# shengjie-chen/simple_image_compression_network

Measured on AMD Instinct MI355X. Metric: Mpixels/s encode+decode (4K RGB), higher is better.
Workload: dtype u8; 1 GPU; 8 x 3840x2160 RGB uint8 images per GPU, eight_layers_net (PARAM weights), BASELINE.json configs[3] shard; transform only (the reference has no coder); images_per_gpu=8, global_images=8, parallelism=image-sharded x1, partition=image i -> rank i mod world (dist.shard_indices)

## Files before the change

include/sicn.h:

```cpp
#ifndef SICN_H
#define SICN_H

#include <stddef.h>
#include <stdint.h>

#ifdef __cplusplus
extern "C" {
#endif

#define SICN_OK 0
#define SICN_EINVAL (-22)
#define SICN_ENOMEM (-12)
#define SICN_ENODEV (-19)
#define SICN_ENOSPC (-28)

typedef struct sicn_layer_desc {
    int32_t K;
    int32_t S;
    int32_t P;
    int32_t IFM_CH;
    int32_t IFM_ROW;
    int32_t IFM_COL;
    int32_t OFM_CH;
    int32_t OFM_ROW;
// ... 44 lines not shown
void sicn_weights_free(sicn_weights *w);

int sicn_conv2d(const sicn_layer_desc *desc, const sicn_weights *w, const uint8_t *in_nhwc,
                uint8_t *out_nhwc, int n_images, void *hip_stream);
int sicn_deconv522(const sicn_layer_desc *desc, const sicn_weights *w, const uint8_t *in_nhwc,
                   uint8_t *out_nhwc, int n_images, void *hip_stream);
int sicn_conv2d_opt(const sicn_layer_desc *desc, const sicn_weights *w, const uint8_t *in_nhwc,
                    uint8_t *out_nhwc, int n_images, const sicn_options *opt, void *hip_stream);
int sicn_deconv522_opt(const sicn_layer_desc *desc, const sicn_weights *w, const uint8_t *in_nhwc,
                       uint8_t *out_nhwc, int n_images, const sicn_options *opt, void *hip_stream);
const char *sicn_kernel_for(const sicn_layer_desc *desc);

int sicn_net_create(const sicn_layer_desc *descs, sicn_weights *const *weights, int n_layers,
                    sicn_net **out);
int sicn_net_create_opt(const sicn_layer_desc *descs, sicn_weights *const *weights, int n_layers,
                        const sicn_options *opt, sicn_net **out);
void sicn_net_free(sicn_net *net);
size_t sicn_net_workspace_bytes(const sicn_net *net, int n_images);
int sicn_net_forward(const sicn_net *net, int first_layer, int last_layer, const uint8_t *in,
                     uint8_t *out, int tap_layer, uint8_t *tap_out, int n_images, void *workspace,
                     size_t workspace_bytes, void *hip_stream);
int sicn_debug_net_columns(const sicn_net *net, int first_layer, int last_layer, int tap_layer, int n_images, int32_t *columns,
                           int32_t *live_outputs);
int sicn_eight_layers_net(const sicn_net *net, const uint8_t *in, uint8_t *out,
                          uint8_t *latent_or_null, int n_images, void *workspace,
                          size_t workspace_bytes, void *hip_stream);

int sicn_net_profile(sicn_net *net, int enable);
int sicn_net_layer_ms(sicn_net *net, int reset, float *ms_sum ,
                      int *launches );

#ifdef __cplusplus
}
#endif
#endif
```

simple_image_compression_network_amd/_lib.py:

```python
from __future__ import annotations

import ctypes
import os
from pathlib import Path

from .config import CLayerDesc

_PKG = Path(__file__).resolve().parent
LIB_PATH = Path(os.environ.get("SICN_LIB", _PKG / "libsicn.so"))

_vp, _i, _sz = ctypes.c_void_p, ctypes.c_int, ctypes.c_size_t


class COptions(ctypes.Structure):
    _fields_ = [(n, ctypes.c_int32) for n in ("struct_bytes", "force_generic", "mfma_shape", "tile_x", "strip_chunks",
                                              "no_phase_layout", "split_n", "wave_tile", "prefetch", "persistent_grid", "split_k", "l7_loader", "l0_form", "gdn_fuse")] + [("reserved", ctypes.c_int32 * 2)]


def make_options(**kw) -> "COptions":
    o = COptions()
    lib().sicn_options_init(ctypes.byref(o))
    for k, v in kw.items():
        if k not in dict(COptions._fields_) or k in ("struct_bytes", "reserved"):
            raise AttributeError(f"sicn_options has no field {k}")
# ... 8 lines not shown
    "sicn_strerror": (ctypes.c_char_p, [_i]),
    "sicn_validate_desc": (_i, [_descp]),
    "sicn_weights_from_finn_tiles": (_i, [_descp, _vp, _i, _vp, ctypes.POINTER(_vp)]),
    "sicn_weights_free": (None, [_vp]),
    "sicn_conv2d": (_i, [_descp, _vp, _vp, _vp, _i, _vp]),
    "sicn_deconv522": (_i, [_descp, _vp, _vp, _vp, _i, _vp]),
    "sicn_kernel_for": (ctypes.c_char_p, [_descp]),
    "sicn_options_init": (None, [ctypes.POINTER(COptions)]),
    "sicn_conv2d_opt": (_i, [_descp, _vp, _vp, _vp, _i, ctypes.POINTER(COptions), _vp]),
    "sicn_deconv522_opt": (_i, [_descp, _vp, _vp, _vp, _i, ctypes.POINTER(COptions), _vp]),
    "sicn_net_create_opt": (_i, [_descp, ctypes.POINTER(_vp), _i, ctypes.POINTER(COptions), ctypes.POINTER(_vp)]),
    "sicn_net_create": (_i, [_descp, ctypes.POINTER(_vp), _i, ctypes.POINTER(_vp)]),
    "sicn_net_free": (None, [_vp]),
    "sicn_net_workspace_bytes": (_sz, [_vp, _i]),
    "sicn_net_forward": (_i, [_vp, _i, _i, _vp, _vp, _i, _vp, _i, _vp, _sz, _vp]),
    "sicn_eight_layers_net": (_i, [_vp, _vp, _vp, _vp, _i, _vp, _sz, _vp]),
    "sicn_net_profile": (_i, [_vp, _i]),
    "sicn_net_layer_ms": (_i, [_vp, _i, ctypes.POINTER(ctypes.c_float), ctypes.POINTER(_i)]),
    "sicn_crop_nhwc": (_i, [_vp, _vp, _i, _i, _i, _i, _i, _i, _vp]),
    "sicn_debug_plan": (_i, [_descp, _i, ctypes.POINTER(COptions), _i, ctypes.POINTER(ctypes.c_int32)]),
    "sicn_debug_xcd_item": (ctypes.c_longlong, [ctypes.c_longlong, ctypes.c_longlong, _i]),
    "sicn_debug_chip": (_i, [ctypes.POINTER(ctypes.c_int32)]),
    "sicn_debug_net_columns": (_i, [_vp, _i, _i, _i, _i, ctypes.POINTER(ctypes.c_int32), ctypes.POINTER(ctypes.c_int32)]),
}


class CodecInfo(ctypes.Structure):
    _fields_ = [(n, ctypes.c_uint32) for n in ("mode", "image_width", "image_height", "lat_w", "lat_h", "lat_c",
                                               "n_symbols", "n_streams", "payload_bytes", "adler32", "stream_symbols")]


class CConvLayerDesc(ctypes.Structure):
    _fields_ = [(n, ctypes.c_int32) for n in ("K", "IFM_CH", "IFM_DIM", "OFM_CH", "OFM_DIM", "SIMD", "PE", "IN_BIT", "IN_SIGNED",
                                              "W_BIT", "W_TILES", "ACC_BIT", "ACC_SIGNED", "OUT_BIT", "activation", "NUM_TH",
                                              "ACT_VAL")]


_cldp = ctypes.POINTER(CConvLayerDesc)
CONVLAYER_ABI = {
    "sicn_convlayer_validate": (_i, [_cldp]),
    "sicn_convlayer_params_create": (_i, [_cldp, _vp, _i, _vp, ctypes.POINTER(_vp)]),
    "sicn_convlayer_params_free": (None, [_vp]),
    "sicn_conv_layer_batch": (_i, [_cldp, _vp, _vp, _vp, _i, _vp]),
    "sicn_conv_layer_batch_kernel": (_i, [_cldp, _vp, _vp, _vp, _i, _i, _vp]),
    "sicn_convlayer_kernel_for": (ctypes.c_char_p, [_cldp]),
}
# ... 201 lines not shown
```

simple_image_compression_network_amd/csrc/k_rgb.hip:

```cpp
#include <cstdlib>

#include <algorithm>

#include "k_l0_common.hpp"

namespace sicn {

template <int NTJ>
__global__ __launch_bounds__(256, 2) void k_l0(const uint8_t *__restrict__ in, uint8_t *__restrict__ out,
                                               const int8_t *__restrict__ w_l0,
                                               const int8_t *__restrict__ bias, int IW, int IH, int OW,
                                               int OH, int tiles_y, int ty_per, int out_layout, uint32_t act_floor)
{
    constexpr int COUT = NTJ * 32;
    constexpr int TB = COUT * KSTEP;
    constexpr int WBYTES = 5 * TB;
    extern __shared__ __attribute__((aligned(16))) uint8_t smem[];
    uint8_t *wl = smem;
    uint8_t *patch0 = smem + WBYTES;
    uint8_t *bias_lds = patch0 + 2 * L0_PATCH;
    uint8_t *raw = bias_lds + 128;

    const int tid = threadIdx.x, lane = tid & 63;
    const int w = __builtin_amdgcn_readfirstlane(tid >> 6);
// ... 127 lines not shown
        const size_t lds = 5 * 128 * KSTEP + 2 * L0_PATCH + 128 + L0_RAW_BYTES;
        hipError_t e = hipFuncSetAttribute((const void *)k_l0<4>, hipFuncAttributeMaxDynamicSharedMemorySize, (int)lds);
        if (e != hipSuccess) return e;
        hipLaunchKernelGGL(k_l0<4>, grid, dim3(256), lds, stream, in, out, w.d_w_l0, w.d_bias, g.IW, g.IH,
                           g.OW, g.OH, p.tiles_y, p.ty_per, out_layout,
                           (relu ? ACT_FLOOR_RELU : ACT_FLOOR_RAW) | (nt_store_wanted((size_t)g.OH * g.OW * g.COUT * n_images) ? ACT_NT_STORE : 0u));
    } else
        return hipErrorInvalidValue;
    return hipGetLastError();
}

constexpr int L7_AUX = 0;
constexpr int L7_PITCH = 36;
constexpr int L7_STEP_PIECES = L7_ROWS * L7_PITCH / 16;
constexpr int L7_AHEAD = 1;
constexpr int L7_RING_PIECES = ((4 * L7_AHEAD + 6) * L7_PITCH + 15) / 16;
constexpr int L7_WGS = 3;
constexpr int L7_RING_POS = L7_RING_PIECES * 16;
constexpr int L7_REGION = L7_RING_PIECES * 1024;
constexpr int L7_STAGE = 2 * 192;
constexpr int L7_X1 = 2 * 256;
constexpr int L7_X2 = 2 * 128;
constexpr int L7_XCH = 5 * L7_X1 + 4 * L7_X2;
constexpr int L7_LDS = 2 * L7_REGION + 4 * L7_STAGE + 1024 + L7_XCH;
constexpr int L7_KSTEPS = 6, L7_MTILES = 2;
static_assert(L7_ROWS * L7_PITCH % 16 == 0 && L7_RING_POS >= (4 * L7_AHEAD + 6) * L7_PITCH, "ring geometry");
static_assert(L7_WGS * L7_LDS <= 160 * 1024 && L7_XCH <= 4096, "three workgroups per CU");

template <int N>
__device__ __forceinline__ void l7_load_rows(uint8_t *patch, uint8_t *scratch, const uint8_t *in_img, int in_img_bytes, int w,
                                             int lane, int per_region, int iy0, int iy_min, int iy_max, int pslot0, int X0,
                                             int IW, const TensorMap &tm)
{
    __amdgpu_buffer_rsrc_t rs = __builtin_amdgcn_make_buffer_rsrc((void *)in_img, 0, in_img_bytes, 0x00020000);
    const int c2 = (lane & 3) ^ ((lane >> 4) & 3);
#pragma unroll
    for (int i = 0; i < N; i++) {
        const int j = w + 4 * i;
        const bool real = j < 2 * per_region;
        const int region = j >= per_region ? 1 : 0, kk = j - region * per_region;
        const int q = kk * 16 + (lane >> 2);
        const int row = q / L7_PITCH, tx = q - row * L7_PITCH;
        const int iy = iy0 + row, ix = X0 - 1 + tx;
        const bool ok = real && tx < TILE_X + 2 && iy >= iy_min && iy < iy_max && ix >= 0 && ix < IW;
        const uint32_t off = ok ? tensor_offset(tm, iy, ix, (uint32_t)(2 * region + (c2 >> 1))) + 16u * (c2 & 1) : OOB;
        int slot = pslot0 + kk;
        slot = slot >= L7_RING_PIECES ? slot - L7_RING_PIECES : slot;
        uint8_t *dst = real ? patch + region * L7_REGION + slot * 1024 : scratch;
        __builtin_amdgcn_raw_ptr_buffer_load_lds(rs, LDS_PTR(dst), 16, off, 0, 0, L7_AUX);
    }
}

__device__ __forceinline__ void l7_body(const uint8_t *__restrict__ in, uint8_t *__restrict__ out, const int8_t *__restrict__ w_l7,
                                        const int8_t *__restrict__ bias, int IW, int IH, int OW, int OH, int steps_y, int y_chunks,
                                        int tiles_x, int n_images, int in_layout, int n_xcd)
{
    constexpr int CIN = 128;
    extern __shared__ __attribute__((aligned(16))) uint8_t smem[];
    uint8_t *patch = smem;
    uint8_t *stage = smem + 2 * L7_REGION;
    uint8_t *scratch = stage + 4 * L7_STAGE;
    uint8_t *xch1 = scratch + 1024;
    uint8_t *xch2 = xch1 + 5 * L7_X1;

    const int tid = threadIdx.x, lane = tid & 63;
    const int w = __builtin_amdgcn_readfirstlane(tid >> 6);
    const int item = xcd_logical_index(tiles_x * y_chunks * n_images, n_xcd);
    if (item < 0) return;
    const int bx = item % tiles_x, by = (item / tiles_x) % y_chunks, img = item / (tiles_x * y_chunks);
    const int X0 = bx * TILE_X;
    const int per = (steps_y + y_chunks - 1) / y_chunks;
    const int s_begin = by * per, s_end = min(steps_y, s_begin + per);
    if (s_begin >= s_end) return;

    const int m = lane & 15, kg = lane >> 4;
    v4i wf[L7_MTILES * L7_KSTEPS];
#pragma unroll
    for (int s = 0; s < L7_MTILES * L7_KSTEPS; s++) wf[s] = *(const v4i *)(w_l7 + (s * 16 + m) * 64 + kg * 16);
    const int b0 = bias[0], b1 = bias[1], b2 = bias[2];

    const int in_img_bytes = IH * IW * CIN;
    const uint8_t *in_img = in + (size_t)img * in_img_bytes;
    uint8_t *out_img = out + (size_t)img * OH * OW * 3;
    const int py = kg >> 1, px = kg & 1;
    uint8_t *my_stage = stage + w * L7_STAGE;
    const bool fast_rows = ((OW * 3) & 3) == 0 && X0 + TILE_X <= IW;

    const int iy_top = 4 * s_begin - 3;
    const int iy_max = min(IH, 4 * s_end + 1);
    const TensorMap tm = tensor_map(in_layout, CIN, IW, IH);
    l7_load_rows<9>(patch, scratch, in_img, in_img_bytes, w, lane, 2 * L7_STEP_PIECES, iy_top, max(iy_top + 2, 0), iy_max, 0, X0,
                    IW, tm);
    int pnext = 2 * L7_STEP_PIECES;
    int ynext = iy_top + 8;
#pragma unroll
    for (int k = 1; k < L7_AHEAD; k++) {
        l7_load_rows<5>(patch, scratch, in_img, in_img_bytes, w, lane, L7_STEP_PIECES, ynext, 0, iy_max, pnext, X0, IW, tm);
        ynext += L7_ROWS;
        pnext += L7_STEP_PIECES;
        pnext = pnext >= L7_RING_PIECES ? pnext - L7_RING_PIECES : pnext;
    }

    auto frag_a = [&](int dx) { return (uint32_t)((4 + w) * L7_PITCH + m + dx); };
    auto frag_s = [&](uint32_t a) { return (uint32_t)((kg & 1) * L7_REGION) + ((((uint32_t)(kg >> 1)) ^ ((a >> 2) & 3u)) << 4); };
    uint32_t fa[3], fs[3];
#pragma unroll
    for (int dx = 0; dx < 3; dx++) {
        fa[dx] = frag_a(dx);
        fs[dx] = frag_s(fa[dx]);
    }
    const int w_below = (w + 1) & 3;
    const uint32_t x1_lane = (uint32_t)lane * 4u, x2_lane = (uint32_t)(px * 16 + m) * 4u;
    int saved[2][3] = {{0, 0, 0}, {0, 0, 0}};
    wait_vmcnt<5 * (L7_AHEAD - 1)>();
    block_barrier();

    int base = L7_RING_POS - L7_ROWS * L7_PITCH;
    for (int s = s_begin - 1; s < s_end; s++) {
        const bool live = s >= s_begin;
        const int par = (s - s_begin) & 1;
        const int Y = 4 * s;
        if (live) {
            l7_load_rows<5>(patch, scratch, in_img, in_img_bytes, w, lane, L7_STEP_PIECES, ynext, 0, iy_max, pnext, X0, IW, tm);
            ynext += L7_ROWS;
        }

        v4i acc[2][L7_MTILES];
#pragma unroll
        for (int c = 0; c < 2; c++) {
            acc[c][0] = v4i{b0, b1, b2, 0};
            acc[c][1] = v4i{0, 0, 0, 0};
#pragma unroll
            for (int dx = 0; dx < 3; dx++) {
                uint32_t slot = (uint32_t)base + fa[dx] + 16u * c;
                slot = min(slot, slot - (uint32_t)L7_RING_POS);
                const uint32_t addr = slot * 64u + fs[dx];
                const v4i p0 = *(const v4i *)(patch + addr);
                const v4i p1 = *(const v4i *)(patch + (addr ^ 32u));
#pragma unroll
                for (int t = 0; t < L7_MTILES; t++) {
                    acc[c][t] = __builtin_amdgcn_mfma_i32_16x16x64_i8(wf[t * L7_KSTEPS + dx * 2 + 0], p0, acc[c][t], 0, 0, 0);
                    acc[c][t] = __builtin_amdgcn_mfma_i32_16x16x64_i8(wf[t * L7_KSTEPS + dx * 2 + 1], p1, acc[c][t], 0, 0, 0);
                }
            }
        }
        {
            uint8_t *x1 = xch1 + (w == 3 ? 3 + par : w) * L7_X1, *x2 = xch2 + w * L7_X2;
#pragma unroll
            for (int c = 0; c < 2; c++) {
                const uint32_t lo = __builtin_amdgcn_perm((uint32_t)acc[c][1][1], (uint32_t)acc[c][1][0], 0x0c0c0400u);
                *(uint32_t *)(x1 + c * 256 + x1_lane) = __builtin_amdgcn_perm((uint32_t)acc[c][1][2], lo, 0x0c040100u);
                *(uint16_t *)(x2 + c * 128 + x2_lane + 2 * py) =
                    (uint16_t)__builtin_amdgcn_perm((uint32_t)acc[c][1][3], (uint32_t)acc[c][0][3], 0x0c0c0400u);
            }
        }
        block_barrier();
        int fin[2][3];
        {
            const int w_above1 = w == 0 ? 3 + (par ^ 1) : w - 1, w_below1 = w_below == 3 ? 3 + par : w_below;
            const uint8_t *x1 = xch1 + (py ? w_below1 : w_above1) * L7_X1, *x2 = xch2 + w_below * L7_X2;
#pragma unroll
            for (int c = 0; c < 2; c++) {
                const uint32_t r1 = *(const uint32_t *)(x1 + c * 256 + x1_lane);
                const uint32_t r2 = *(const uint32_t *)(x2 + c * 128 + x2_lane);
                const uint32_t above = py ? 0u : r1, below = py ? r1 : r2;
// ... 7 lines not shown
            }
        }
        const int gy = Y + w_below;
        if (fast_rows) {
#pragma unroll
            for (int c = 0; c < 2; c++) {
                const uint32_t v = pack4_relu7(fin[c][0], fin[c][1], fin[c][2], 0);
                uint8_t *d = my_stage + py * 192 + (2 * (16 * c + m) + px) * 3;
                d[0] = (uint8_t)v;
                d[1] = (uint8_t)(v >> 8);
                d[2] = (uint8_t)(v >> 16);
            }
            asm volatile("s_waitcnt lgkmcnt(0)" ::: "memory");
            __amdgpu_buffer_rsrc_t ro = __builtin_amdgcn_make_buffer_rsrc((void *)out_img, 0, OH * OW * 3, 0x00020000);
#pragma unroll
            for (int k = 0; k < 2; k++) {
                const int idx = k * 64 + lane;
                const int row = idx >= 48 ? 1 : 0, col = idx - 48 * row;
                const bool ok = live && idx < 96 && gy < IH;
                const uint32_t v = *(const uint32_t *)(my_stage + (idx < 96 ? idx : 0) * 4);
                const uint32_t off = ok ? (uint32_t)(((2 * gy + row) * OW + 2 * X0) * 3 + col * 4) : OOB;
                __builtin_amdgcn_raw_buffer_store_b32(v, ro, off, 0, 0);
            }
            wait_vmcnt<2 + 7 * (L7_AHEAD - 1)>();
        } else {
#pragma unroll
            for (int c = 0; c < 2; c++) {
                const int gx = X0 + 16 * c + m;
                if (live && gy < IH && gx < IW) {
                    const uint32_t v = pack4_relu7(fin[c][0], fin[c][1], fin[c][2], 0);
                    uint8_t *dst = out_img + ((size_t)(2 * gy + py) * OW + 2 * gx + px) * 3;
                    dst[0] = (uint8_t)v;
                    dst[1] = (uint8_t)(v >> 8);
                    dst[2] = (uint8_t)(v >> 16);
                }
            }
            wait_vmcnt<0>();
        }
        block_barrier();
        base += L7_ROWS * L7_PITCH;
        base = base >= L7_RING_POS ? base - L7_RING_POS : base;
        if (live) {
            pnext += L7_STEP_PIECES;
            pnext = pnext >= L7_RING_PIECES ? pnext - L7_RING_PIECES : pnext;
        }
    }
    wait_vmcnt<0>();
}
__global__ __launch_bounds__(256, L7_WGS) void k_l7(const uint8_t *__restrict__ in, uint8_t *__restrict__ out, const int8_t *__restrict__ w_l7,
                                                    const int8_t *__restrict__ bias, int IW, int IH, int OW, int OH, int steps_y, int y_chunks,
                                                    int tiles_x, int n_images, int in_layout, int n_xcd)
{
    l7_body(in, out, w_l7, bias, IW, IH, OW, OH, steps_y, y_chunks, tiles_x, n_images, in_layout, n_xcd);
}

size_t l7_bytes(int cin) { return (size_t)L7_MTILES * L7_KSTEPS * 16 * 64 * (cin / 128); }

void pack_l7(const int8_t *w_okc, int cin, int8_t *dst)
{
    for (int tile = 0; tile < L7_MTILES; tile++)
        for (int dx = 0; dx < 3; dx++)
            for (int half = 0; half < 2; half++)
                for (int row = 0; row < 16; row++) {
                    const int g = row >> 2, r = row & 3, py = g >> 1, px = g & 1;
                    int ky, c;
                    if (r < 3) {
                        ky = tile == 0 ? 2 - py : (py ? 3 : 0);
                        c = r;
                    } else {
                        ky = 4;
                        c = py ? (tile == 0 ? 2 : -1) : tile;
                    }
                    const int kx = 2 * dx - px;
                    int8_t *t = dst + ((((size_t)tile * 3 + dx) * 2 + half) * 16 + row) * 64;
                    for (int b = 0; b < 64; b++) {
                        const int kg = b >> 4, ch = 64 * (kg & 1) + 32 * half + 16 * (kg >> 1) + (b & 15);
                        t[b] = (c >= 0 && kx >= 0 && kx < 5) ? w_okc[(size_t)c * 25 * cin + (ky * 5 + kx) * cin + ch] : 0;
                    }
                }
}

hipError_t launch_l7(const LayerGeom &g, const sicn_weights &w, const uint8_t *in, uint8_t *out,
                     int n_images, hipStream_t stream, int in_layout, const sicn_options &o, const ChipGeom &chip)
{
    if (g.CIN != 128 || g.COUT != 3) return hipErrorInvalidValue;
    if ((size_t)g.IH * g.IW * g.CIN >= (size_t)OOB) return hipErrorInvalidValue;
    if ((size_t)g.OH * g.OW * 3 >= (size_t)OOB) return hipErrorInvalidValue;
    const L7Plan p = plan_l7(g.IW, g.IH, n_images, o.strip_chunks, chip);
    const size_t lds = L7_LDS;
    const dim3 grid(p.grid_x);
    hipError_t e = hipFuncSetAttribute((const void *)k_l7, hipFuncAttributeMaxDynamicSharedMemorySize, (int)lds);
    if (e != hipSuccess) return e;
    hipLaunchKernelGGL(k_l7, grid, dim3(256), lds, stream, in, out, w.d_w_l7, w.d_bias, g.IW, g.IH, g.OW, g.OH, p.steps_y, p.y_chunks,
                       p.tiles_x, n_images, in_layout, chip.n_xcd);
    return hipGetLastError();
}

}
```

simple_image_compression_network_amd/csrc/sicn_abi.hip:

```cpp
#include <array>
#include <atomic>
#include <cmath>
#include <cstdio>
#include <cstdlib>
#include <cstring>
#include <memory>
#include <mutex>
#include <new>
#include <vector>

#include "sicn_gdn_internal.h"
#include "sicn_internal.h"
#include "sicn_live.h"
#include "sicn_weights_io.h"

using namespace sicn;

namespace sicn {
static int env_int(const char *name)
{
    const char *e = getenv(name);
    return (e && *e) ? atoi(e) : 0;
}
template <int32_t... V> static bool one_of(int32_t v) { return ((v == V) || ...); }
// ... 122 lines not shown
    if (d->transposed) {
        if (d->OFM_ROW != 2 * d->IFM_ROW || d->OFM_COL != 2 * d->IFM_COL) return SICN_EINVAL;
    } else if (d->OFM_ROW != (d->IFM_ROW + 1) / 2 || d->OFM_COL != (d->IFM_COL + 1) / 2)
        return SICN_EINVAL;
    return SICN_OK;
}

namespace {
enum : unsigned { GROUP = 1u << 1, PHASE = 1u << 2 };

struct LaunchArgs {
    const LayerGeom &g;
    const sicn_weights &w;
    const uint8_t *in;
    uint8_t *out;
    int n_images;
    hipStream_t stream;
    int in_layout, out_layout;
    const sicn_options &o;
    const ChipGeom &chip;
    const sicn_gdn *gdn;
    unsigned long long *deal;
    int columns;
};

struct Family {
    KernelKind kind;
    const char *name;
    int transposed;
    bool (*shape)(int cin, int cout, int transposed);
    unsigned reads, writes;
    bool rgb_sink;
    bool pre_relu;
    bool (*upload_images)(const int8_t *w_okc, sicn_weights &w);
    hipError_t (*launch)(const LaunchArgs &a, bool *act_done);
    void (*plan)(const LayerGeom &g, int n_images, const sicn_options &o, const ChipGeom &chip, int32_t out[12]);
    bool (*deals)(const LayerGeom &g, int n_images, const sicn_options &o, const ChipGeom &chip);
};

template <class Pack>
bool upload_image(size_t bytes, int8_t **dev, Pack pack)
{
    std::vector<int8_t> s(bytes);
    pack(s.data());
    return upload(s.data(), s.size(), dev);
}
// ... 1 lines not shown
bool l0_shape(int cin, int cout, int) { return cin == 3 && cout == 128; }
bool l0_images(const int8_t *k, sicn_weights &w)
{
    return upload_image(l0_bytes(w.cout), &w.d_w_l0, [&](int8_t *s) { pack_l0(k, w.cout, s); }) &&
           upload_image(l0g_bytes(), &w.d_w_l0g, [&](int8_t *s) { pack_l0g(k, s); });
}
hipError_t l0_launch(const LaunchArgs &a, bool *act_done)
{
    if (a.gdn && a.o.gdn_fuse != 1 && a.w.d_w_l0g && a.gdn->d_gamma_mfma) {
        *act_done = true;
        return launch_l0_gdn(a.g, a.w, *a.gdn, a.in, a.out, a.n_images, a.stream, a.out_layout, a.o, a.chip);
    }
    return launch_l0(a.g, a.w, a.in, a.out, a.n_images, a.stream, a.out_layout, a.o, a.chip, a.gdn == nullptr);
}
void l0_plan(const LayerGeom &g, int n_images, const sicn_options &o, const ChipGeom &chip, int32_t out[12])
{
    const L0Plan p = plan_l0(g.OW, g.OH, n_images, false, o.strip_chunks, chip);
    out[7] = p.tiles_x; out[8] = p.y_chunks; out[9] = n_images; out[10] = p.y_chunks; out[11] = p.ty_per;
}

bool l7_shape(int cin, int cout, int) { return cin == 128 && cout == 3; }
bool l7_images(const int8_t *k, sicn_weights &w)
{
    return upload_image(l7_bytes(w.cin), &w.d_w_l7, [&](int8_t *s) { pack_l7(k, w.cin, s); });
}
hipError_t l7_launch(const LaunchArgs &a, bool *)
{
    return launch_l7(a.g, a.w, a.in, a.out, a.n_images, a.stream, a.in_layout, a.o, a.chip);
}
void l7_plan(const LayerGeom &g, int n_images, const sicn_options &o, const ChipGeom &chip, int32_t out[12])
{
    const L7Plan p = plan_l7(g.IW, g.IH, n_images, o.strip_chunks, chip);
    out[7] = (int)p.grid_x; out[8] = 1; out[9] = 1; out[10] = p.y_chunks;
}

bool mfma_images(const int8_t *k, sicn_weights &w)
{
    bool ok = upload_image(mfma16_stream_bytes(w.cin, w.cout), &w.d_w_mfma16,
                           [&](int8_t *s) { pack_mfma16_stream(k, w.cin, w.cout, w.transposed, s); });
    if (ok && w.transposed && mfma16x_deconv_stream_bytes(w.cin, w.cout))
        ok = upload_image(mfma16x_deconv_stream_bytes(w.cin, w.cout), &w.d_w_mfma16x,
                          [&](int8_t *s) { pack_mfma16x_deconv_stream(k, w.cin, w.cout, s); });
    return ok;
}
hipError_t mfma_launch(const LaunchArgs &a, bool *)
{
    return launch_mfma16(a.g, a.w, a.in, a.out, a.n_images, a.stream, a.in_layout, a.out_layout, a.o, a.chip, a.gdn == nullptr, a.deal,
                         a.columns);
}
void mfma_plan(const LayerGeom &g, int n_images, const sicn_options &o, const ChipGeom &chip, int32_t out[12])
{
// ... 38 lines not shown
}
const Family &layer_family(const sicn_layer_desc &d, const sicn_options &o, bool has_gdn)
{
    const Family &f = pick_family(d, o);
    return (has_gdn && !f.pre_relu) ? GENERIC : f;
}
}

extern "C" const char *sicn_kernel_for(const sicn_layer_desc *d)
{
    return sicn_validate_desc(d) ? "invalid" : pick_family(*d, default_options()).name;
}

extern "C" void sicn_weights_free(sicn_weights *w)
{
    if (!w) return;
    if (w->d_w_okc) (void)hipFree(w->d_w_okc);
    if (w->d_bias) (void)hipFree(w->d_bias);
    if (w->d_w_mfma16) (void)hipFree(w->d_w_mfma16);
    if (w->d_w_mfma16x) (void)hipFree(w->d_w_mfma16x);
    if (w->d_w_l0) (void)hipFree(w->d_w_l0);
    if (w->d_w_l0g) (void)hipFree(w->d_w_l0g);
    if (w->d_w_l7) (void)hipFree(w->d_w_l7);
    if (w->d_w_any) (void)hipFree(w->d_w_any);
    delete w;
}

static int weights_from_okc(int cin, int cout, int transposed, std::vector<int8_t> w_okc, const int8_t *bias, sicn_weights **out)
{
    sicn_weights *w = new (std::nothrow) sicn_weights();
    if (!w) return SICN_ENOMEM;
    w->cin = cin;
    w->cout = cout;
    w->transposed = transposed;
    bool ok = upload(w_okc.data(), w_okc.size(), &w->d_w_okc);
    try {
        std::vector<int8_t> b(((size_t)cout + 15) / 16 * 16 + 16, 0);
        for (int i = 0; i < cout; i++) b[i] = bias[i];
        ok = ok && upload(b.data(), b.size(), &w->d_bias);
        sicn_layer_desc d{};
        d.IFM_CH = cin;
        d.OFM_CH = cout;
        d.transposed = transposed;
        const Family &f = pick_family(d, sicn_options{});
        if (ok && f.upload_images) ok = f.upload_images(w_okc.data(), *w);
        w->h_bias.assign(bias, bias + cout);
// ... 18 lines not shown
    if (word_bytes != 1 && word_bytes != 2 && word_bytes != 4 && word_bytes != 8) return SICN_EINVAL;
    if (d->SIMD * 4 > word_bytes * 8) return SICN_EINVAL;
    const int cin = d->IFM_CH, cout = d->OFM_CH, kk = 25 * cin;
    std::vector<int8_t> w_okc;
    try {
        w_okc.resize((size_t)cout * kk);
    } catch (const std::bad_alloc &) { return SICN_ENOMEM; }
    decode_finn_tiles(m_weights, word_bytes, 4, d->SIMD, d->PE, d->W_TILES, kk, cout, w_okc.data());
    return weights_from_okc(cin, cout, d->transposed, std::move(w_okc), bias, out);
}

static int link_layout(const sicn_layer_desc &p, const sicn_layer_desc &c, const sicn_options &o, bool p_gdn, bool c_gdn)
{
    const Family &fc = layer_family(c, o, c_gdn);
    const unsigned common = layer_family(p, o, p_gdn).writes & fc.reads;
    const bool phase_ok = o.no_phase_layout == 0 || (o.no_phase_layout == 2 && !fc.rgb_sink);
    if ((common & PHASE) && phase_ok) return 2;
    if (common & GROUP) return 1;
    return 0;
}

static int run_layer(const sicn_layer_desc *d, const sicn_weights *w, const uint8_t *in, uint8_t *out,
                     int n_images, hipStream_t stream, int want_transposed, const sicn_options &o, int in_layout = 0,
                     int out_layout = 0, const sicn_gdn *gdn = nullptr, unsigned long long *deal = nullptr, int columns = 8)
{
    int rc = sicn_validate_desc(d);
    if (rc) return rc;
    if (!w || !in || !out || n_images < 0) return SICN_EINVAL;
    if (want_transposed >= 0 && d->transposed != want_transposed) return SICN_EINVAL;
    if (w->cin != d->IFM_CH || w->cout != d->OFM_CH || w->transposed != d->transposed) return SICN_EINVAL;
    if (n_images == 0) return SICN_OK;
    if (n_images > 65535) return SICN_EINVAL;
    if (gdn && gdn->channels != d->OFM_CH) return SICN_EINVAL;
    const LayerGeom g = geom_of(*d);
    ChipGeom chip;
    if ((rc = chip_geom(&chip)) != SICN_OK) return rc;
    bool act_done = false;
    const LaunchArgs args{g, *w, in, out, n_images, stream, in_layout, out_layout, o, chip, gdn, deal, columns};
    hipError_t e = layer_family(*d, o, gdn != nullptr).launch(args, &act_done);
    if (act_done) gdn = nullptr;
    if (e == hipSuccess && gdn) e = launch_gdn(*gdn, out, out_layout, d->OFM_ROW, d->OFM_COL, n_images, stream);
    if (e == hipErrorInvalidValue) return SICN_EINVAL;
    return e == hipSuccess ? SICN_OK : SICN_ENODEV;
}

extern "C" int sicn_conv2d(const sicn_layer_desc *d, const sicn_weights *w, const uint8_t *in, uint8_t *out,
                           int n_images, void *hip_stream)
{
    return run_layer(d, w, in, out, n_images, (hipStream_t)hip_stream, 0, default_options());
}

extern "C" int sicn_conv2d_opt(const sicn_layer_desc *d, const sicn_weights *w, const uint8_t *in, uint8_t *out,
                               int n_images, const sicn_options *opt, void *hip_stream)
{
    sicn_options o;
    int rc = resolve_options(opt, &o);
    return rc ? rc : run_layer(d, w, in, out, n_images, (hipStream_t)hip_stream, 0, o);
}

extern "C" int sicn_deconv522(const sicn_layer_desc *d, const sicn_weights *w, const uint8_t *in,
                              uint8_t *out, int n_images, void *hip_stream)
// ... 142 lines not shown
{
    if (net->live[(size_t)l].nj >= live::COLS) return live::COLS;
    const Family &f = layer_family(net->descs[(size_t)l], net->opt, false);
    const bool wide = (f.kind == KK_MFMA_CONV || f.kind == KK_MFMA_DECONV) &&
                      plan_mfma(geom_of(net->descs[(size_t)l]), n_images, net->opt, chip).family == 2;
    return live::columns(net->live, l, first, last, tap_layer, wide);
}

extern "C" int sicn_debug_net_columns(const sicn_net *net, int first, int last, int tap_layer, int n_images, int32_t *columns,
                                      int32_t *live_outputs)
{
    if (!net || !columns || !live_outputs || n_images <= 0) return SICN_EINVAL;
    const int n_layers = (int)net->descs.size();
    if (first < 0 || last >= n_layers || first > last) return SICN_EINVAL;
    ChipGeom chip;
    if (int rc = chip_geom(&chip)) return rc;
    for (int l = 0; l < n_layers; l++) {
        columns[l] = call_columns(net, l, first, last, tap_layer, n_images, chip);
        live_outputs[l] = live::live_outputs(net->live, l, first, last, tap_layer);
    }
    return SICN_OK;
}

extern "C" int sicn_net_forward(const sicn_net *net, int first, int last, const uint8_t *in, uint8_t *out,
                                int tap_layer, uint8_t *tap_out, int n_images, void *workspace,
                                size_t workspace_bytes, void *hip_stream)
{
    if (!net || !in || !out || n_images < 0) return SICN_EINVAL;
    const int n_layers = (int)net->descs.size();
    if (first < 0 || last >= n_layers || first > last) return SICN_EINVAL;
    if (tap_layer >= 0 && (tap_layer < first || tap_layer > last || !tap_out)) return SICN_EINVAL;
    if (n_images == 0) return SICN_OK;
    const size_t slot = pingpong_slot_bytes(net, n_images);
    if (last > first && (!workspace || workspace_bytes < 2 * slot)) return SICN_ENOSPC;
    hipStream_t stream = (hipStream_t)hip_stream;
    uint8_t *pp[2] = {(uint8_t *)workspace, (uint8_t *)workspace + slot};
    unsigned long long *deal_base = nullptr;
    ChipGeom chip;
    if (int rc = chip_geom(&chip)) return rc;
    {
        bool any_deal = false;
        for (int l = first; l <= last && !any_deal; l++) {
            const Family &f = pick_family(net->descs[l], net->opt);
            any_deal = f.deals && f.deals(geom_of(net->descs[l]), n_images, net->opt, chip);
        }
        if (any_deal && workspace && workspace_bytes >= 2 * slot + deal_bytes(net) && !debug_env().no_deal) {
            deal_base = (unsigned long long *)((uint8_t *)workspace + 2 * slot);
            if (launch_zero_words(deal_base, deal_bytes(net) / sizeof(unsigned long long), stream) != hipSuccess) return SICN_ENODEV;
        }
    }
    const uint8_t *cur = in;
    int cur_layout = 0;
    int slot0 = -1;
    if (net->profile.load(std::memory_order_acquire)) {
        const int need = last - first + 1;
        const int at = net->ev_next.fetch_add(need, std::memory_order_relaxed);
        if (at + need <= sicn_net::EV_RING) slot0 = at;
    }
    int cols_before = live::COLS;
    for (int l = first; l <= last; l++) {
        const int cols = call_columns(net, l, first, last, tap_layer, n_images, chip);
        const int variant = 2 * (cols_before < live::COLS) + (cols < live::COLS);
        const sicn_weights *wl = variant ? net->derived[l][(size_t)variant] : net->weights[l];
        if (!wl) return SICN_EINVAL;
        cols_before = cols;
        uint8_t *dst = (l == last) ? out : (l == tap_layer ? tap_out : pp[(l - first) & 1]);
        const int out_layout = (l < last && l != tap_layer)
                                   ? link_layout(net->descs[l], net->descs[l + 1], net->opt, net->gdn[l] != nullptr, net->gdn[l + 1] != nullptr)
                                   : 0;
        const int ev = slot0 >= 0 ? slot0 + (l - first) : -1;
        if (ev >= 0) {
            net->ev_layer[ev].store(-1, std::memory_order_relaxed);
            if (hipEventRecord(net->ev_begin[ev], stream) != hipSuccess) return SICN_ENODEV;
        }
        int rc = run_layer(&net->descs[l], wl, cur, dst, n_images, stream, -1, net->opt, cur_layout, out_layout,
                           net->gdn[l], deal_base ? deal_base + (size_t)l * DEAL_WORDS : nullptr, cols);
        if (rc) return rc;
        if (ev >= 0) {
            if (hipEventRecord(net->ev_end[ev], stream) != hipSuccess) return SICN_ENODEV;
            net->ev_layer[ev].store(l, std::memory_order_release);
        }
        if (l == tap_layer && tap_out != dst) {
            if (hipMemcpyAsync(tap_out, dst, out_bytes(net->descs[l]) * (size_t)n_images, hipMemcpyDeviceToDevice,
                               stream) != hipSuccess)
                return SICN_ENODEV;
        }
        cur = dst;
        cur_layout = out_layout;
    }
    return SICN_OK;
}

extern "C" int sicn_eight_layers_net(const sicn_net *net, const uint8_t *in, uint8_t *out, uint8_t *latent,
                                     int n_images, void *workspace, size_t workspace_bytes, void *hip_stream)
{
    if (!net) return SICN_EINVAL;
    const int n = (int)net->descs.size();
    const int tap = latent ? 3 : -1;
    if (latent && n < 4) return SICN_EINVAL;
// ... 191 lines not shown
```

simple_image_compression_network_amd/csrc/sicn_internal.h:

```cpp
#pragma once
#include <hip/hip_runtime.h>
#include <stddef.h>
#include <stdint.h>

#include <vector>

#include "../../include/sicn.h"
#include "sicn_plan.h"

namespace sicn {

constexpr int TILE_Y = 8;
constexpr int PATCH_Y = TILE_Y + 2;
constexpr int KSTEP = 32;

enum KernelKind : int { KK_GENERIC = 0, KK_MFMA_CONV, KK_MFMA_DECONV, KK_L0_RGB, KK_L7_RGB, KK_MFMA_CONV_ANY, KK_MFMA_DECONV_ANY };

struct LayerGeom {
    int IW, IH, CIN, OW, OH, COUT, transposed;
};

inline LayerGeom geom_of(const sicn_layer_desc &d)
{
    return LayerGeom{d.IFM_ROW, d.IFM_COL, d.IFM_CH, d.OFM_ROW, d.OFM_COL, d.OFM_CH, d.transposed};
}

}

struct sicn_ragged_coder;
struct sicn_ragged_cut;
struct sicn_ragged_rect;

struct sicn_weights {
    int cin, cout, transposed;
    int8_t *d_w_okc;
    int8_t *d_bias;
    int8_t *d_w_mfma16;
    int8_t *d_w_mfma16x;
    int8_t *d_w_l0;
    int8_t *d_w_l0g;
    int8_t *d_w_l7;
    int8_t *d_w_any;
    std::vector<int8_t> h_w_okc, h_bias;
};

namespace sicn {

constexpr int DEAL_MAX_WORKGROUPS = WIDE_DEAL_MAX_WORKGROUPS;
constexpr int DEAL_WORDS = WIDE_DEAL_MAX_XCDS + DEAL_MAX_WORKGROUPS;
hipError_t launch_zero_words(unsigned long long *p, size_t words, hipStream_t stream);

struct MfmaPlan {
    int family;
    int tile_x;
    int split_n;
    unsigned grid_x, grid_y, grid_z;
    int deal;
};
MfmaPlan plan_mfma(const LayerGeom &g, int n_images, const sicn_options &o, const ChipGeom &chip);
const sicn_options &default_options();
struct DebugEnv { int no_deal; };
const DebugEnv &debug_env();

int chip_geom(ChipGeom *out);

hipError_t launch_generic(const LayerGeom &g, const sicn_weights &w, const uint8_t *in, uint8_t *out,
                          int n_images, hipStream_t stream, bool relu = true);
hipError_t launch_crop_nhwc(const uint8_t *src, uint8_t *dst, int n, int hs, int ws, int h, int w, int c, hipStream_t stream);
hipError_t launch_mfma16(const LayerGeom &g, const sicn_weights &w, const uint8_t *in, uint8_t *out,
                         int n_images, hipStream_t stream, int in_layout, int out_layout, const sicn_options &o, const ChipGeom &chip,
                         bool relu = true, unsigned long long *deal = nullptr, int columns = 8);
bool wide_supported(const LayerGeom &g);
size_t mfma16x_deconv_stream_bytes(int cin, int cout);
void pack_mfma16x_deconv_stream(const int8_t *w_okc, int cin, int cout, int8_t *dst);
hipError_t launch_wide(const LayerGeom &g, const sicn_weights &w, const uint8_t *in, uint8_t *out, int n_images, hipStream_t stream,
                       int in_layout, int out_layout, bool relu, int grid_cap, const ChipGeom &chip, unsigned long long *deal = nullptr,
                       int columns = 8);
const void *wide_live_kernel(int transposed, bool nt_store, int columns);
bool pipelined_supported(const LayerGeom &g, int tile_x);
hipError_t launch_pipelined(const LayerGeom &g, const sicn_weights &w, const uint8_t *in, uint8_t *out, int n_images,
                            hipStream_t stream, int in_layout, int out_layout, bool relu, int tile_x, bool split_channels,
                            const ChipGeom &chip);
hipError_t launch_l0(const LayerGeom &g, const sicn_weights &w, const uint8_t *in, uint8_t *out,
                     int n_images, hipStream_t stream, int out_layout, const sicn_options &o, const ChipGeom &chip, bool relu = true);
hipError_t launch_l7(const LayerGeom &g, const sicn_weights &w, const uint8_t *in, uint8_t *out,
                     int n_images, hipStream_t stream, int in_layout, const sicn_options &o, const ChipGeom &chip);

bool mfma_supported(int cin, int cout, int transposed);
size_t mfma16_stream_bytes(int cin, int cout);
void pack_mfma16_stream(const int8_t *w_okc, int cin, int cout, int transposed, int8_t *dst);

bool any_supported(int cin, int cout, int transposed);
size_t any_bytes(int cin, int cout);
void pack_any(const int8_t *w_okc, int cin, int cout, int8_t *dst);
hipError_t launch_any(const LayerGeom &g, const sicn_weights &w, const uint8_t *in, uint8_t *out, int n_images, hipStream_t stream,
                      bool relu = true);

struct RaggedCoderView {
    int n_images;
    const void *rows_host, *d_rows;
    size_t row_bytes;
    uint64_t ws_bytes;
};
void ragged_coder_view(const sicn_ragged_coder *coder, RaggedCoderView *v);

int ragged_cut_layout(const int32_t *src_w, const int32_t *src_h, const sicn_ragged_rect *rects, int channels,
                      const uint64_t *src_offset_or_null, int n_images, int image, int64_t out[4]);
int ragged_cut_create(const int32_t *src_w, const int32_t *src_h, const sicn_ragged_rect *rects, int channels,
                      const uint64_t *src_offset_or_null, int n_images, sicn_ragged_cut **out);
int ragged_cut_run(const sicn_ragged_cut *cut, const uint8_t *src, uint8_t *dst, void *hip_stream);

size_t l0_bytes(int cout);
void pack_l0(const int8_t *w_okc, int cout, int8_t *dst);
size_t l0g_bytes();
void pack_l0g(const int8_t *w_okc, int8_t *dst);
size_t l7_bytes(int cin);
void pack_l7(const int8_t *w_okc, int cin, int8_t *dst);

}
```

Measured before the change: 23390 Mpixels/s.

## Add half-channel L7 kernel variant when upstream writes only four live columns

Templates the final RGB layer kernel on the number of 64-channel input halves it reads. When the previous layer produces only the live columns (<=4) in a non-NHWC layout, the L7 kernel loads and multiplies only the first half, using a separately packed half weight image. The intent is to cut L7 input loads, LDS footprint and MFMA count on dead channels. It adds a second weight upload and a new swizzle path that must match the producer's layout.

```diff
diff --git a/include/sicn.h b/include/sicn.h
--- a/include/sicn.h
+++ b/include/sicn.h
@@ -90,6 +90,7 @@
                      size_t workspace_bytes, void *hip_stream);
 int sicn_debug_net_columns(const sicn_net *net, int first_layer, int last_layer, int tap_layer, int n_images, int32_t *columns,
                            int32_t *live_outputs);
+int sicn_debug_net_input_halves(const sicn_net *net, int first_layer, int last_layer, int tap_layer, int n_images, int32_t *halves);
 int sicn_eight_layers_net(const sicn_net *net, const uint8_t *in, uint8_t *out,
                           uint8_t *latent_or_null, int n_images, void *workspace,
                           size_t workspace_bytes, void *hip_stream);
diff --git a/simple_image_compression_network_amd/_lib.py b/simple_image_compression_network_amd/_lib.py
--- a/simple_image_compression_network_amd/_lib.py
+++ b/simple_image_compression_network_amd/_lib.py
@@ -54,6 +54,7 @@
     "sicn_debug_xcd_item": (ctypes.c_longlong, [ctypes.c_longlong, ctypes.c_longlong, _i]),
     "sicn_debug_chip": (_i, [ctypes.POINTER(ctypes.c_int32)]),
     "sicn_debug_net_columns": (_i, [_vp, _i, _i, _i, _i, ctypes.POINTER(ctypes.c_int32), ctypes.POINTER(ctypes.c_int32)]),
+    "sicn_debug_net_input_halves": (_i, [_vp, _i, _i, _i, _i, ctypes.POINTER(ctypes.c_int32)]),
 }
 
 
diff --git a/simple_image_compression_network_amd/csrc/k_rgb.hip b/simple_image_compression_network_amd/csrc/k_rgb.hip
--- a/simple_image_compression_network_amd/csrc/k_rgb.hip
+++ b/simple_image_compression_network_amd/csrc/k_rgb.hip
@@ -173,23 +173,33 @@
 constexpr int L7_X1 = 2 * 256;
 constexpr int L7_X2 = 2 * 128;
 constexpr int L7_XCH = 5 * L7_X1 + 4 * L7_X2;
-constexpr int L7_LDS = 2 * L7_REGION + 4 * L7_STAGE + 1024 + L7_XCH;
-constexpr int L7_KSTEPS = 6, L7_MTILES = 2;
+constexpr int L7_MTILES = 2;
+template <int KH>
+struct L7Form {
+    static_assert(KH == 1 || KH == 2, "one or two 64-channel halves");
+    static constexpr int LDS = KH * L7_REGION + 4 * L7_STAGE + 1024 + L7_XCH;
+    static constexpr int KSTEPS = 3 * KH;
+    static constexpr int PRO_N = (KH * 2 * L7_STEP_PIECES + 3) / 4;
+    static constexpr int STEP_N = (KH * L7_STEP_PIECES + 3) / 4;
+    static constexpr int WGS = L7_WGS;
+};
 static_assert(L7_ROWS * L7_PITCH % 16 == 0 && L7_RING_POS >= (4 * L7_AHEAD + 6) * L7_PITCH, "ring geometry");
-static_assert(L7_WGS * L7_LDS <= 160 * 1024 && L7_XCH <= 4096, "three workgroups per CU");
-
-template <int N>
+static_assert(L7Form<2>::WGS * L7Form<2>::LDS <= 160 * 1024 && L7Form<1>::WGS * L7Form<1>::LDS <= 160 * 1024 && L7_XCH <= 4096,
+              "workgroups per CU");
+static_assert(L7Form<2>::LDS == 53248 && L7Form<2>::PRO_N == 9 && L7Form<2>::STEP_N == 5, "KH = 2 is the kernel it was");
+
+template <int N, int KH>
 __device__ __forceinline__ void l7_load_rows(uint8_t *patch, uint8_t *scratch, const uint8_t *in_img, int in_img_bytes, int w,
                                              int lane, int per_region, int iy0, int iy_min, int iy_max, int pslot0, int X0,
                                              int IW, const TensorMap &tm)
 {
     __amdgpu_buffer_rsrc_t rs = __builtin_amdgcn_make_buffer_rsrc((void *)in_img, 0, in_img_bytes, 0x00020000);
-    const int c2 = (lane & 3) ^ ((lane >> 4) & 3);
+    const int c2 = KH == 2 ? (lane & 3) ^ ((lane >> 4) & 3) : 2 * ((lane & 1) ^ ((lane >> 4) & 1)) + ((lane >> 1) & 1);
 #pragma unroll
     for (int i = 0; i < N; i++) {
         const int j = w + 4 * i;
-        const bool real = j < 2 * per_region;
-        const int region = j >= per_region ? 1 : 0, kk = j - region * per_region;
+        const bool real = j < KH * per_region;
+        const int region = (KH == 2 && j >= per_region) ? 1 : 0, kk = j - region * per_region;
         const int q = kk * 16 + (lane >> 2);
         const int row = q / L7_PITCH, tx = q - row * L7_PITCH;
         const int iy = iy0 + row, ix = X0 - 1 + tx;
@@ -202,6 +212,7 @@
     }
 }
 
+template <int KH>
 __device__ __forceinline__ void l7_body(const uint8_t *__restrict__ in, uint8_t *__restrict__ out, const int8_t *__restrict__ w_l7,
                                         const int8_t *__restrict__ bias, int IW, int IH, int OW, int OH, int steps_y, int y_chunks,
                                         int tiles_x, int n_images, int in_layout, int n_xcd)
@@ -209,7 +220,8 @@
     constexpr int CIN = 128;
     extern __shared__ __attribute__((aligned(16))) uint8_t smem[];
     uint8_t *patch = smem;
-    uint8_t *stage = smem + 2 * L7_REGION;
+    using F = L7Form<KH>;
+    uint8_t *stage = smem + KH * L7_REGION;
     uint8_t *scratch = stage + 4 * L7_STAGE;
     uint8_t *xch1 = scratch + 1024;
     uint8_t *xch2 = xch1 + 5 * L7_X1;
@@ -225,9 +237,9 @@
     if (s_begin >= s_end) return;
 
     const int m = lane & 15, kg = lane >> 4;
-    v4i wf[L7_MTILES * L7_KSTEPS];
-#pragma unroll
-    for (int s = 0; s < L7_MTILES * L7_KSTEPS; s++) wf[s] = *(const v4i *)(w_l7 + (s * 16 + m) * 64 + kg * 16);
+    v4i wf[L7_MTILES * F::KSTEPS];
+#pragma unroll
+    for (int s = 0; s < L7_MTILES * F::KSTEPS; s++) wf[s] = *(const v4i *)(w_l7 + (s * 16 + m) * 64 + kg * 16);
     const int b0 = bias[0], b1 = bias[1], b2 = bias[2];
 
     const int in_img_bytes = IH * IW * CIN;
@@ -240,20 +252,23 @@
     const int iy_top = 4 * s_begin - 3;
     const int iy_max = min(IH, 4 * s_end + 1);
     const TensorMap tm = tensor_map(in_layout, CIN, IW, IH);
-    l7_load_rows<9>(patch, scratch, in_img, in_img_bytes, w, lane, 2 * L7_STEP_PIECES, iy_top, max(iy_top + 2, 0), iy_max, 0, X0,
+    l7_load_rows<F::PRO_N, KH>(patch, scratch, in_img, in_img_bytes, w, lane, 2 * L7_STEP_PIECES, iy_top, max(iy_top + 2, 0), iy_max, 0, X0,
                     IW, tm);
     int pnext = 2 * L7_STEP_PIECES;
     int ynext = iy_top + 8;
 #pragma unroll
     for (int k = 1; k < L7_AHEAD; k++) {
-        l7_load_rows<5>(patch, scratch, in_img, in_img_bytes, w, lane, L7_STEP_PIECES, ynext, 0, iy_max, pnext, X0, IW, tm);
+        l7_load_rows<F::STEP_N, KH>(patch, scratch, in_img, in_img_bytes, w, lane, L7_STEP_PIECES, ynext, 0, iy_max, pnext, X0, IW, tm);
         ynext += L7_ROWS;
         pnext += L7_STEP_PIECES;
         pnext = pnext >= L7_RING_PIECES ? pnext - L7_RING_PIECES : pnext;
     }
 
     auto frag_a = [&](int dx) { return (uint32_t)((4 + w) * L7_PITCH + m + dx); };
-    auto frag_s = [&](uint32_t a) { return (uint32_t)((kg & 1) * L7_REGION) + ((((uint32_t)(kg >> 1)) ^ ((a >> 2) & 3u)) << 4); };
+    auto frag_s = [&](uint32_t a) {
+        return KH == 2 ? (uint32_t)((kg & 1) * L7_REGION) + ((((uint32_t)(kg >> 1)) ^ ((a >> 2) & 3u)) << 4)
+                       : (2u * (uint32_t)(kg & 1) + (((uint32_t)(kg >> 1)) ^ ((a >> 2) & 1u))) << 4;
+    };
     uint32_t fa[3], fs[3];
 #pragma unroll
     for (int dx = 0; dx < 3; dx++) {
@@ -263,7 +278,7 @@
     const int w_below = (w + 1) & 3;
     const uint32_t x1_lane = (uint32_t)lane * 4u, x2_lane = (uint32_t)(px * 16 + m) * 4u;
     int saved[2][3] = {{0, 0, 0}, {0, 0, 0}};
-    wait_vmcnt<5 * (L7_AHEAD - 1)>();
+    wait_vmcnt<F::STEP_N * (L7_AHEAD - 1)>();
     block_barrier();
 
     int base = L7_RING_POS - L7_ROWS * L7_PITCH;
@@ -272,7 +287,7 @@
         const int par = (s - s_begin) & 1;
         const int Y = 4 * s;
         if (live) {
-            l7_load_rows<5>(patch, scratch, in_img, in_img_bytes, w, lane, L7_STEP_PIECES, ynext, 0, iy_max, pnext, X0, IW, tm);
+            l7_load_rows<F::STEP_N, KH>(patch, scratch, in_img, in_img_bytes, w, lane, L7_STEP_PIECES, ynext, 0, iy_max, pnext, X0, IW, tm);
             ynext += L7_ROWS;
         }
 
@@ -287,11 +302,17 @@
                 slot = min(slot, slot - (uint32_t)L7_RING_POS);
                 const uint32_t addr = slot * 64u + fs[dx];
                 const v4i p0 = *(const v4i *)(patch + addr);
-                const v4i p1 = *(const v4i *)(patch + (addr ^ 32u));
-#pragma unroll
-                for (int t = 0; t < L7_MTILES; t++) {
-                    acc[c][t] = __builtin_amdgcn_mfma_i32_16x16x64_i8(wf[t * L7_KSTEPS + dx * 2 + 0], p0, acc[c][t], 0, 0, 0);
-                    acc[c][t] = __builtin_amdgcn_mfma_i32_16x16x64_i8(wf[t * L7_KSTEPS + dx * 2 + 1], p1, acc[c][t], 0, 0, 0);
+                if constexpr (KH == 2) {
+                    const v4i p1 = *(const v4i *)(patch + (addr ^ 32u));
+#pragma unroll
+                    for (int t = 0; t < L7_MTILES; t++) {
+                        acc[c][t] = __builtin_amdgcn_mfma_i32_16x16x64_i8(wf[t * F::KSTEPS + dx * 2 + 0], p0, acc[c][t], 0, 0, 0);
+                        acc[c][t] = __builtin_amdgcn_mfma_i32_16x16x64_i8(wf[t * F::KSTEPS + dx * 2 + 1], p1, acc[c][t], 0, 0, 0);
+                    }
+                } else {
+#pragma unroll
+                    for (int t = 0; t < L7_MTILES; t++)
+                        acc[c][t] = __builtin_amdgcn_mfma_i32_16x16x64_i8(wf[t * F::KSTEPS + dx], p0, acc[c][t], 0, 0, 0);
                 }
             }
         }
@@ -345,7 +366,7 @@
                 const uint32_t off = ok ? (uint32_t)(((2 * gy + row) * OW + 2 * X0) * 3 + col * 4) : OOB;
                 __builtin_amdgcn_raw_buffer_store_b32(v, ro, off, 0, 0);
             }
-            wait_vmcnt<2 + 7 * (L7_AHEAD - 1)>();
+            wait_vmcnt<2 + (F::STEP_N + 2) * (L7_AHEAD - 1)>();
         } else {
 #pragma unroll
             for (int c = 0; c < 2; c++) {
@@ -370,14 +391,16 @@
     }
     wait_vmcnt<0>();
 }
-__global__ __launch_bounds__(256, L7_WGS) void k_l7(const uint8_t *__restrict__ in, uint8_t *__restrict__ out, const int8_t *__restrict__ w_l7,
+template <int KH>
+__global__ __launch_bounds__(256, L7Form<KH>::WGS) void k_l7(const uint8_t *__restrict__ in, uint8_t *__restrict__ out, const int8_t *__restrict__ w_l7,
                                                     const int8_t *__restrict__ bias, int IW, int IH, int OW, int OH, int steps_y, int y_chunks,
                                                     int tiles_x, int n_images, int in_layout, int n_xcd)
 {
-    l7_body(in, out, w_l7, bias, IW, IH, OW, OH, steps_y, y_chunks, tiles_x, n_images, in_layout, n_xcd);
-}
-
-size_t l7_bytes(int cin) { return (size_t)L7_MTILES * L7_KSTEPS * 16 * 64 * (cin / 128); }
+    l7_body<KH>(in, out, w_l7, bias, IW, IH, OW, OH, steps_y, y_chunks, tiles_x, n_images, in_layout, n_xcd);
+}
+
+size_t l7_bytes(int cin) { return (size_t)L7_MTILES * L7Form<2>::KSTEPS * 16 * 64 * (cin / 128); }
+size_t l7_half_bytes() { return (size_t)L7_MTILES * L7Form<1>::KSTEPS * 16 * 64; }
 
 void pack_l7(const int8_t *w_okc, int cin, int8_t *dst)
 {
@@ -403,20 +426,49 @@
                 }
 }
 
+void pack_l7_half(const int8_t *w_okc, int8_t *dst)
+{
+    for (int tile = 0; tile < L7_MTILES; tile++)
+        for (int dx = 0; dx < 3; dx++)
+            for (int row = 0; row < 16; row++) {
+                const int g = row >> 2, r = row & 3, py = g >> 1, px = g & 1;
+                int ky, c;
+                if (r < 3) {
+                    ky = tile == 0 ? 2 - py : (py ? 3 : 0);
+                    c = r;
+                } else {
+                    ky = 4;
+                    c = py ? (tile == 0 ? 2 : -1) : tile;
+                }
+                const int kx = 2 * dx - px;
+                int8_t *t = dst + (((size_t)tile * 3 + dx) * 16 + row) * 64;
+                for (int b = 0; b < 64; b++)
+                    t[b] = (c >= 0 && kx >= 0 && kx < 5) ? w_okc[(size_t)c * 25 * 128 + (ky * 5 + kx) * 128 + b] : 0;
+            }
+}
+
+template <int KH>
+static hipError_t launch_l7_form(const LayerGeom &g, const int8_t *w_img, const sicn_weights &w, const uint8_t *in, uint8_t *out, int n_images,
+                                 hipStream_t stream, int in_layout, const L7Plan &p, const ChipGeom &chip)
+{
+    const size_t lds = L7Form<KH>::LDS;
+    hipError_t e = hipFuncSetAttribute((const void *)k_l7<KH>, hipFuncAttributeMaxDynamicSharedMemorySize, (int)lds);
+    if (e != hipSuccess) return e;
+    hipLaunchKernelGGL(k_l7<KH>, dim3(p.grid_x), dim3(256), lds, stream, in, out, w_img, w.d_bias, g.IW, g.IH, g.OW, g.OH, p.steps_y, p.y_chunks,
+                       p.tiles_x, n_images, in_layout, chip.n_xcd);
+    return hipGetLastError();
+}
+
 hipError_t launch_l7(const LayerGeom &g, const sicn_weights &w, const uint8_t *in, uint8_t *out,
-                     int n_images, hipStream_t stream, int in_layout, const sicn_options &o, const ChipGeom &chip)
+                     int n_images, hipStream_t stream, int in_layout, const sicn_options &o, const ChipGeom &chip, int halves)
 {
     if (g.CIN != 128 || g.COUT != 3) return hipErrorInvalidValue;
+    if (halves == 1 && (in_layout == LAYOUT_NHWC || !w.d_w_l7_half)) return hipErrorInvalidValue;
     if ((size_t)g.IH * g.IW * g.CIN >= (size_t)OOB) return hipErrorInvalidValue;
     if ((size_t)g.OH * g.OW * 3 >= (size_t)OOB) return hipErrorInvalidValue;
     const L7Plan p = plan_l7(g.IW, g.IH, n_images, o.strip_chunks, chip);
-    const size_t lds = L7_LDS;
-    const dim3 grid(p.grid_x);
-    hipError_t e = hipFuncSetAttribute((const void *)k_l7, hipFuncAttributeMaxDynamicSharedMemorySize, (int)lds);
-    if (e != hipSuccess) return e;
-    hipLaunchKernelGGL(k_l7, grid, dim3(256), lds, stream, in, out, w.d_w_l7, w.d_bias, g.IW, g.IH, g.OW, g.OH, p.steps_y, p.y_chunks,
-                       p.tiles_x, n_images, in_layout, chip.n_xcd);
-    return hipGetLastError();
-}
-
-}
+    return halves == 1 ? launch_l7_form<1>(g, w.d_w_l7_half, w, in, out, n_images, stream, in_layout, p, chip)
+                       : launch_l7_form<2>(g, w.d_w_l7, w, in, out, n_images, stream, in_layout, p, chip);
+}
+
+}
diff --git a/simple_image_compression_network_amd/csrc/sicn_abi.hip b/simple_image_compression_network_amd/csrc/sicn_abi.hip
--- a/simple_image_compression_network_amd/csrc/sicn_abi.hip
+++ b/simple_image_compression_network_amd/csrc/sicn_abi.hip
@@ -168,6 +168,7 @@
     const sicn_gdn *gdn;
     unsigned long long *deal;
     int columns;
+    int columns_in;
 };
 
 struct Family {
@@ -215,11 +216,13 @@
 bool l7_shape(int cin, int cout, int) { return cin == 128 && cout == 3; }
 bool l7_images(const int8_t *k, sicn_weights &w)
 {
-    return upload_image(l7_bytes(w.cin), &w.d_w_l7, [&](int8_t *s) { pack_l7(k, w.cin, s); });
-}
+    return upload_image(l7_bytes(w.cin), &w.d_w_l7, [&](int8_t *s) { pack_l7(k, w.cin, s); }) &&
+           upload_image(l7_half_bytes(), &w.d_w_l7_half, [&](int8_t *s) { pack_l7_half(k, s); });
+}
+bool l7_reads_one_half(int columns_in, int in_layout) { return columns_in <= 4 && in_layout != 0; }
 hipError_t l7_launch(const LaunchArgs &a, bool *)
 {
-    return launch_l7(a.g, a.w, a.in, a.out, a.n_images, a.stream, a.in_layout, a.o, a.chip);
+    return launch_l7(a.g, a.w, a.in, a.out, a.n_images, a.stream, a.in_layout, a.o, a.chip, l7_reads_one_half(a.columns_in, a.in_layout) ? 1 : 2);
 }
 void l7_plan(const LayerGeom &g, int n_images, const sicn_options &o, const ChipGeom &chip, int32_t out[12])
 {
@@ -304,6 +307,7 @@
     if (w->d_w_l0) (void)hipFree(w->d_w_l0);
     if (w->d_w_l0g) (void)hipFree(w->d_w_l0g);
     if (w->d_w_l7) (void)hipFree(w->d_w_l7);
+    if (w->d_w_l7_half) (void)hipFree(w->d_w_l7_half);
     if (w->d_w_any) (void)hipFree(w->d_w_any);
     delete w;
 }
@@ -368,7 +372,8 @@
 
 static int run_layer(const sicn_layer_desc *d, const sicn_weights *w, const uint8_t *in, uint8_t *out,
                      int n_images, hipStream_t stream, int want_transposed, const sicn_options &o, int in_layout = 0,
-                     int out_layout = 0, const sicn_gdn *gdn = nullptr, unsigned long long *deal = nullptr, int columns = 8)
+                     int out_layout = 0, const sicn_gdn *gdn = nullptr, unsigned long long *deal = nullptr, int columns = 8,
+                     int columns_in = 8)
 {
     int rc = sicn_validate_desc(d);
     if (rc) return rc;
@@ -382,7 +387,7 @@
     ChipGeom chip;
     if ((rc = chip_geom(&chip)) != SICN_OK) return rc;
     bool act_done = false;
-    const LaunchArgs args{g, *w, in, out, n_images, stream, in_layout, out_layout, o, chip, gdn, deal, columns};
+    const LaunchArgs args{g, *w, in, out, n_images, stream, in_layout, out_layout, o, chip, gdn, deal, columns, columns_in};
     hipError_t e = layer_family(*d, o, gdn != nullptr).launch(args, &act_done);
     if (act_done) gdn = nullptr;
     if (e == hipSuccess && gdn) e = launch_gdn(*gdn, out, out_layout, d->OFM_ROW, d->OFM_COL, n_images, stream);
@@ -571,6 +576,26 @@
     return SICN_OK;
 }
 
+extern "C" int sicn_debug_net_input_halves(const sicn_net *net, int first, int last, int tap_layer, int n_images, int32_t *halves)
+{
+    if (!net || !halves || n_images <= 0) return SICN_EINVAL;
+    const int n_layers = (int)net->descs.size();
+    if (first < 0 || last >= n_layers || first > last) return SICN_EINVAL;
+    ChipGeom chip;
+    if (int rc = chip_geom(&chip)) return rc;
+    for (int l = 0; l < n_layers; l++) halves[l] = 2;
+    int cols_before = live::COLS, cur_layout = 0;
+    for (int l = first; l <= last; l++) {
+        const bool l7 = layer_family(net->descs[l], net->opt, net->gdn[l] != nullptr).kind == KK_L7_RGB;
+        if (l7 && l7_reads_one_half(cols_before, cur_layout)) halves[l] = 1;
+        cols_before = call_columns(net, l, first, last, tap_layer, n_images, chip);
+        cur_layout = (l < last && l != tap_layer)
+                         ? link_layout(net->descs[l], net->descs[l + 1], net->opt, net->gdn[l] != nullptr, net->gdn[l + 1] != nullptr)
+                         : 0;
+    }
+    return SICN_OK;
+}
+
 extern "C" int sicn_net_forward(const sicn_net *net, int first, int last, const uint8_t *in, uint8_t *out,
                                 int tap_layer, uint8_t *tap_out, int n_images, void *workspace,
                                 size_t workspace_bytes, void *hip_stream)
@@ -612,6 +637,7 @@
         const int variant = 2 * (cols_before < live::COLS) + (cols < live::COLS);
         const sicn_weights *wl = variant ? net->derived[l][(size_t)variant] : net->weights[l];
         if (!wl) return SICN_EINVAL;
+        const int cols_in = cols_before;
         cols_before = cols;
         uint8_t *dst = (l == last) ? out : (l == tap_layer ? tap_out : pp[(l - first) & 1]);
         const int out_layout = (l < last && l != tap_layer)
@@ -623,7 +649,7 @@
             if (hipEventRecord(net->ev_begin[ev], stream) != hipSuccess) return SICN_ENODEV;
         }
         int rc = run_layer(&net->descs[l], wl, cur, dst, n_images, stream, -1, net->opt, cur_layout, out_layout,
-                           net->gdn[l], deal_base ? deal_base + (size_t)l * DEAL_WORDS : nullptr, cols);
+                           net->gdn[l], deal_base ? deal_base + (size_t)l * DEAL_WORDS : nullptr, cols, cols_in);
         if (rc) return rc;
         if (ev >= 0) {
             if (hipEventRecord(net->ev_end[ev], stream) != hipSuccess) return SICN_ENODEV;
diff --git a/simple_image_compression_network_amd/csrc/sicn_internal.h b/simple_image_compression_network_amd/csrc/sicn_internal.h
--- a/simple_image_compression_network_amd/csrc/sicn_internal.h
+++ b/simple_image_compression_network_amd/csrc/sicn_internal.h
@@ -40,6 +40,7 @@
     int8_t *d_w_l0;
     int8_t *d_w_l0g;
     int8_t *d_w_l7;
+    int8_t *d_w_l7_half;
     int8_t *d_w_any;
     std::vector<int8_t> h_w_okc, h_bias;
 };
@@ -84,7 +85,7 @@
 hipError_t launch_l0(const LayerGeom &g, const sicn_weights &w, const uint8_t *in, uint8_t *out,
                      int n_images, hipStream_t stream, int out_layout, const sicn_options &o, const ChipGeom &chip, bool relu = true);
 hipError_t launch_l7(const LayerGeom &g, const sicn_weights &w, const uint8_t *in, uint8_t *out,
-                     int n_images, hipStream_t stream, int in_layout, const sicn_options &o, const ChipGeom &chip);
+                     int n_images, hipStream_t stream, int in_layout, const sicn_options &o, const ChipGeom &chip, int halves = 2);
 
 bool mfma_supported(int cin, int cout, int transposed);
 size_t mfma16_stream_bytes(int cin, int cout);
@@ -116,5 +117,7 @@
 void pack_l0g(const int8_t *w_okc, int8_t *dst);
 size_t l7_bytes(int cin);
 void pack_l7(const int8_t *w_okc, int cin, int8_t *dst);
+size_t l7_half_bytes();
+void pack_l7_half(const int8_t *w_okc, int8_t *dst);
 
 }
```

Measured after the change: 24970 Mpixels/s, median of 6. +6.7%, better.
